# sokunmin/Improved-Body-Parts

Measured on AMD Instinct MI355X. Metric: end-to-end images/sec at 512×512, higher is better.
Workload: dtype f16; 1 GPU; configs[2]+forward: 512x512, flip=on, host->HBM ingest + 4-stage IMHN forward (fp16) + full HIP pafprocess (NMS + limb line-integral + assembly); launch=hipGraph replay, parallelism=image-sharded x1

## Files before the change

improved-body-parts_amd/csrc/posepaf_conv_own.hip:

```cpp
#include <hip/hip_fp16.h>
#include <hip/hip_runtime.h>

#include <atomic>
#include <cstdint>
#include <cstdlib>
#include <type_traits>

#include "../../include/posepaf.h"

namespace {

typedef _Float16 half8_t __attribute__((ext_vector_type(8)));
typedef _Float16 half4_t __attribute__((ext_vector_type(4)));
typedef float float4_t __attribute__((ext_vector_type(4)));

constexpr int BM = 256;
constexpr int NTHREADS = 512;
constexpr int SUB = 1024;

struct ConvParams {
    const _Float16 *x, *w, *bias, *extra, *extra2;
    _Float16 *y, *y2;
    const void *zero;
    int N, H, W, C, K, R, pad, dil, Ho, Wo;
// ... 2 lines not shown
    float *csum;
    int ldy;
    int ldx = 0;
    long M;
    int mode;
    int up;
    float slope;
    int stagger;
    int dbg;
};

__device__ __forceinline__ void lds_dma16(const void *gsrc, unsigned char *lds_wave_base) {
    __builtin_amdgcn_global_load_lds((const __attribute__((address_space(1))) void *)gsrc,
                                     (__attribute__((address_space(3))) void *)lds_wave_base, 16, 0, 0);
}

__device__ __forceinline__ void lds_dma16_buf(__amdgpu_buffer_rsrc_t rsrc, unsigned voffset, unsigned soffset, unsigned char *lds_wave_base) {
    __builtin_amdgcn_raw_ptr_buffer_load_lds(rsrc, (__attribute__((address_space(3))) void *)lds_wave_base, 16, (int)voffset, (int)soffset, 0, 0);
}

typedef float float2_t __attribute__((ext_vector_type(2)));
typedef _Float16 half2_t __attribute__((ext_vector_type(2)));

template <int MODE, int PT, int CT, bool SUMS = false, typename PixelOf>
__device__ __forceinline__ void epilogue_body(const float4_t (&acc)[PT][CT], const ConvParams &p, int lane, int nbase,
                                              PixelOf pixel_of, bool do_store, float *sums_row = nullptr) {
    static_assert(CT % 2 == 0, "channel tiles are finished in pairs");
    const int g = lane >> 4, odd = g & 1, cbase = (g & ~1) * 4;
    const float2_t slope2 = float2_t{p.slope, p.slope};
#pragma unroll
    for (int jp = 0; jp < CT; jp += 2) {
        float csum[8] = {0.f, 0.f, 0.f, 0.f, 0.f, 0.f, 0.f, 0.f};
        const int co = nbase + (jp + odd) * 16 + cbase;
        const half8_t bv = *reinterpret_cast<const half8_t *>(p.bias + co);
        float2_t b2[4];
#pragma unroll
        for (int e = 0; e < 4; e++) b2[e] = float2_t{(float)bv[2 * e], (float)bv[2 * e + 1]};
#pragma unroll
        for (int i = 0; i < PT; i++) {
            float v[8];
#pragma unroll
            for (int e = 0; e < 4; e++) {
                const float a0 = acc[i][jp][e], a1 = acc[i][jp + 1][e];
                const auto sw = __builtin_amdgcn_permlane16_swap(__float_as_uint(a0), __float_as_uint(a1), false, false);
                v[e] = __builtin_bit_cast(float, (unsigned)sw[0]);
                v[4 + e] = __builtin_bit_cast(float, (unsigned)sw[1]);
            }
            const long m = pixel_of(i);
            if (m >= 0) {
                const long o = m * p.K + co;
                half8_t ev = half8_t{0, 0, 0, 0, 0, 0, 0, 0}, ev2 = half8_t{0, 0, 0, 0, 0, 0, 0, 0};
                if (MODE) ev = *reinterpret_cast<const half8_t *>(p.extra + o);
                if (MODE >= 3) ev2 = *reinterpret_cast<const half8_t *>(p.extra2 + o);
                half8_t out, out2;
// ... 72 lines not shown
                v[e] = __builtin_bit_cast(float, (unsigned)sw[0]);
                v[4 + e] = __builtin_bit_cast(float, (unsigned)sw[1]);
            }
            const long m = pixel_of(i);
            keep[i] = half8_t{0, 0, 0, 0, 0, 0, 0, 0};
            if (m >= 0) {
                const half8_t ev = pre[i][jp / 2], ev2 = pre2[i][jp / 2];
                half8_t out, out2;
#pragma unroll
                for (int e = 0; e < 4; e++) {
                    float2_t t = float2_t{v[2 * e], v[2 * e + 1]} + b2[e];
                    const float2_t x = float2_t{(float)ev[2 * e], (float)ev[2 * e + 1]};
                    if (MODE == 1 || MODE == 4) t += x;
                    const float2_t u = t * slope2;
                    t = float2_t{fmaxf(t[0], u[0]), fmaxf(t[1], u[1])};
                    if (MODE == 2) t += x;
                    out[2 * e] = (_Float16)t[0];
                    out[2 * e + 1] = (_Float16)t[1];
                    if (MODE == 4 || MODE == 5) {
                        out2[2 * e] = (_Float16)((float)out[2 * e] + (float)ev2[2 * e]);
                        out2[2 * e + 1] = (_Float16)((float)out[2 * e + 1] + (float)ev2[2 * e + 1]);
                    }
                }
                *reinterpret_cast<half8_t *>(p.y + (m * p.ldy + co)) = out;
                if (MODE == 4 || MODE == 5) *reinterpret_cast<half8_t *>(p.y2 + (m * p.K + co)) = out2;
                keep[i] = (MODE == 4 || MODE == 5) ? out2 : out;
            }
        }
        if (POOL && PT >= 2) {
            constexpr int CB = PT >= 2 ? PT / 2 : 1;
#pragma unroll
            for (int cb = 0; cb < CB; cb++) {
                const half8_t vert = __builtin_elementwise_max(keep[cb], keep[CB + cb]);
                const half8_t pm = __builtin_elementwise_max(vert, lane_xor1(vert));
                if (!(lane & 1)) *reinterpret_cast<half8_t *>(pool + ((pool_base + cb * 8 + ((lane & 15) >> 1)) * p.K + co)) = pm;
            }
        }
    }
}

template <int PT, int CT, typename PixelOf>
__device__ __forceinline__ void epilogue_store(const float4_t (&acc)[PT][CT], const ConvParams &p, int lane, int nbase,
                                               PixelOf pixel_of, bool do_store, float *sums_row = nullptr) {
    if (nbase >= p.K) return;
    if (sums_row) epilogue_body<0, PT, CT, true>(acc, p, lane, nbase, pixel_of, do_store, sums_row);
    else if (p.mode == 0) epilogue_body<0, PT, CT>(acc, p, lane, nbase, pixel_of, do_store);
    else if (p.mode == 1) epilogue_body<1, PT, CT>(acc, p, lane, nbase, pixel_of, do_store);
    else if (p.mode == 2) epilogue_body<2, PT, CT>(acc, p, lane, nbase, pixel_of, do_store);
    else if (p.mode == 3) epilogue_body<3, PT, CT>(acc, p, lane, nbase, pixel_of, do_store);
    else epilogue_body<4, PT, CT>(acc, p, lane, nbase, pixel_of, do_store);
}

template <int PT, int CT, typename PixelOfQ>
__device__ __forceinline__ void epilogue_fullline_probe(const float4_t (&acc)[PT][CT], const ConvParams &p, int lane, int nbase,
                                                        PixelOfQ pixel_of_q) {
    const int co = nbase + (lane >> 3) * 8;
    const half8_t bv = *reinterpret_cast<const half8_t *>(p.bias + co);
#pragma unroll
    for (int jp = 0; jp < CT; jp += 2)
#pragma unroll
        for (int i = 0; i < PT; i++) {
            const long o = pixel_of_q(i * 16 + (jp >> 1) * 8 + (lane & 7)) * p.K + co;
            half8_t out;
#pragma unroll
            for (int e = 0; e < 8; e++) {
                float t = (e < 4 ? acc[i][jp][e] : acc[i][jp + 1][e - 4]) + (float)bv[e];
                t = t > 0.f ? t : t * p.slope;
                out[e] = (_Float16)t;
            }
            *reinterpret_cast<half8_t *>(p.y + o) = out;
        }
}

template <int N>
__device__ __forceinline__ void wait_lgkmcnt() {
    asm volatile("s_waitcnt lgkmcnt(%0)" ::"n"(N) : "memory");
}
__device__ __forceinline__ void mfma_acc(float4_t &c, const half8_t &a, const half8_t &b) {
    asm volatile("v_mfma_f32_16x16x32_f16 %0, %1, %2, %0" : "+v"(c) : "v"(a), "v"(b));
}
template <int OFF>
__device__ __forceinline__ void lds_read16(half8_t &dst, unsigned lds_addr) {
    asm volatile("ds_read_b128 %0, %1 offset:%2" : "=v"(dst) : "v"(lds_addr), "n"(OFF));
}

template <int N>
__device__ __forceinline__ void wait_vmcnt() {
    asm volatile("s_waitcnt vmcnt(%0)" ::"n"(N) : "memory");
}

template <int BN>
__global__ __launch_bounds__(NTHREADS) void k_conv_igemm(const ConvParams p) {
    constexpr int WN = BN / 64;
    constexpr int WM = 8 / WN;
    constexpr int PM = BM / WM;
    constexpr int PT = PM / 16;
    constexpr int CT = 4;
    constexpr int A_BYTES = BM * 32 * 2;
    constexpr int B_BYTES = BN * 32 * 2;
    constexpr int PBUF = A_BYTES + B_BYTES;
    constexpr int NBUF = 4;
    constexpr int BL = BN == 256 ? 2 : 1;
// ... 96 lines not shown
        __builtin_amdgcn_s_setprio(1);
#pragma unroll
        for (int i = 0; i < PT; i++)
#pragma unroll
            for (int j = 0; j < CT; j++) acc[i][j] = __builtin_amdgcn_mfma_f32_16x16x32_f16(wf[j], xf[i], acc[i][j], 0, 0, 0);
        __builtin_amdgcn_s_setprio(0);
        __builtin_amdgcn_s_barrier();
    }
    if (grp == 0) __builtin_amdgcn_s_barrier();

    epilogue_store<PT, CT>(acc, p, lane, n0 + wn * 64, [&](int i) -> long {
        const long m = m0 + wm * PM + i * 16 + (lane & 15);
        if (m >= p.M) return -1;
        if (!p.up_out) return m;
        const int n = (int)(m / HoWo), rem = (int)(m - (long)n * HoWo);
        const int oy_ = rem / p.Wo, ox_ = rem - oy_ * p.Wo;
        return ((long)n * (2 * p.Ho) + 2 * oy_ + p.py) * (2 * p.Wo) + 2 * ox_ + p.px;
    }, true);
}

constexpr int TP = 512;
constexpr int HALO_RES_SUMS = 2048;
constexpr int HALO_DBG_BITS = HALO_RES_SUMS - 1;

struct HaloParams {
    int TW, TH, lgTW;
    int tiles_x, tiles;
    int HWp, nhalo, npieces;
    int gimg, hrows;
    int tps;
};

__device__ unsigned long long g_conv_clk[8 * 512];

template <int BN, int MASK, int LGTW, int PH = -1, int D = 1>
__global__ __launch_bounds__(NTHREADS) void k_conv3x3_halo(const ConvParams p, const HaloParams hp) {
    constexpr int NT = PH < 0 ? 9 : 4;
    static_assert(D == 1 || PH < 0, "the collapsed upsample form has no dilation");
    constexpr int TW = 1 << LGTW, HWp = TW + 2 * D, TH = TP / TW;
    constexpr int dbg = MASK & HALO_DBG_BITS;
    constexpr int WN = BN / 64;
    constexpr int WM = 8 / WN;
    constexpr int PM = TP / WM;
    constexpr int PT = PM / 16;
    constexpr int CT = 4;
    constexpr int WB = BN * 32 * 2;
// ... 81 lines not shown

    const int ncb = p.C / 32;
    const int np = ncb * NT;
    int st_cb = 0, st_tap = 0;
    int st_slot = 0;
    int slot_cur = 0;
    auto stage_w = [&]() {
        lds_dma16_buf(rsrc_of(bw_lo, bw_hi, bw_n), woff, (unsigned)((st_tap * p.C + st_cb * 32) * 2), s_w + st_slot * WB + wave * SUB);
        if (++st_slot == NW) st_slot = 0;
        if (++st_tap == NT) {
            st_tap = 0;
            ++st_cb;
        }
    };
    auto stage_halo = [&](int t, int cb, int buf) {
        lds_dma16_buf(rsrc_of(bx_lo, bx_hi, nx), (unsigned)hsrc[t], (unsigned)(cb * 64), s_halo + buf * halo_bytes + (t * 8 + wave) * SUB);
    };

    const int wfrag = (lane & 15) * 64 + (((lane >> 4) * 16) ^ (((lane & 15) >> 3) << 5));
    const int rows_before = (wm * PM) >> LGTW;
    const int hb0 = ((rows_before + (hp.gimg > 1 ? 2 * (rows_before / p.H) : 0)) * HWp + ((wm * PM) & (TW - 1)) + (lane & 15)) * 64 +
                    (lane >> 4) * 16;
    const unsigned lds_halo = (unsigned)(uintptr_t)(__attribute__((address_space(3))) unsigned char *)s_halo;
    const unsigned lds_w = (unsigned)(uintptr_t)(__attribute__((address_space(3))) unsigned char *)s_w + wn * 4 * SUB;
    unsigned R[4][2];
    auto set_R = [&]() {
#pragma unroll
        for (int k = 0; k < 4; k++) {
            const int M = hb0 + k * 64;
            const unsigned a = lds_halo + (unsigned)(M ^ ((M >> 3) & 32));
            R[k][0] = a;
            R[k][1] = a ^ 32u;
        }
    };
    auto flip_R = [&](int to_buf) {
        const unsigned d = to_buf ? (unsigned)halo_bytes : (unsigned)-halo_bytes;
#pragma unroll
        for (int k = 0; k < 4; k++) R[k][0] += d, R[k][1] += d;
    };
    auto xread = [&](auto TAP, auto I, half8_t &dst) {
        constexpr int tap = decltype(TAP)::value, i = decltype(I)::value;
        constexpr int trow = PH < 0 ? tap / 3 : (PH >> 1) + (tap >> 1), tcol = PH < 0 ? D * (tap % 3) : (PH & 1) + (tap & 1);
        constexpr int Cpix = trow * HWp + tcol + ((i * 16) >> LGTW) * HWp + ((i * 16) & (TW - 1));
        constexpr int C = Cpix * 64, k = Cpix & 3, Chi = C & ~255, f = (Chi >> 8) & 1;
        static_assert(Chi < 65536, "16-bit DS offset");
        lds_read16<Chi>(dst, R[k][f]);
    };

    auto stage_first = [&]() {
        st_cb = 0, st_tap = 0, st_slot = 0;
#pragma unroll
        for (int t = 0; t < NPW; t++)
            if (t < 4 || (t == 4 && p4) || (t == 5 && p5) || (t == 6 && p6)) stage_halo(t, 0, 0);
        for (int q = 0; q < AHEAD && q < np; q++) stage_w();
    };
    unsigned long long acc_t[6] = {0, 0, 0, 0, 0, 0}, t_prev = 0;
    auto stamp = [&](int k) {
        if (dbg & 1024) {
            const unsigned long long t = __builtin_amdgcn_s_memtime();
            if (k >= 0) acc_t[k] += t - t_prev;
            t_prev = t;
        }
    };
    int id = next_tile(blockIdx.x);
    if (id >= total_ids) return;
    for (int z = (int)(blockIdx.x >> 3) * p.stagger / (int)((gridDim.x + 7) >> 3); z > 0; z--) __builtin_amdgcn_s_sleep(127);
    stage_first();
  while (true) {
    const int c_img = n_img, c_ty0 = ty0, c_tx0 = tx0, c_n0 = n0, c_tile = t_idx;
    float4_t acc[PT][CT];
#pragma unroll
    for (int i = 0; i < PT; i++)
#pragma unroll
        for (int j = 0; j < CT; j++) acc[i][j] = float4_t{0.f, 0.f, 0.f, 0.f};
    stamp(-1);
    wait_vmcnt<0>();
    __builtin_amdgcn_s_barrier();
    stamp(0);
    slot_cur = 0;
    half8_t wf[CT], xf[PT];
    set_R();
    lds_read16<0>(wf[0], lds_w + wfrag);
    lds_read16<SUB>(wf[1], lds_w + wfrag);
    using T0 = std::integral_constant<int, 0>;
    xread(T0{}, std::integral_constant<int, 0>{}, xf[0]);
    xread(T0{}, std::integral_constant<int, 1>{}, xf[1]);
    xread(T0{}, std::integral_constant<int, 2>{}, xf[2]);
    xread(T0{}, std::integral_constant<int, 3>{}, xf[3]);
    xread(T0{}, std::integral_constant<int, 4>{}, xf[4]);
    xread(T0{}, std::integral_constant<int, 5>{}, xf[5]);
    xread(T0{}, std::integral_constant<int, 6>{}, xf[6]);
    xread(T0{}, std::integral_constant<int, 7>{}, xf[7]);
// ... 51 lines not shown
                mfma_acc(acc[i][1], wf[1], xf[i]);
            }
        };
        tile_a(std::integral_constant<int, 0>{});
        tile_a(std::integral_constant<int, 1>{});
        tile_a(std::integral_constant<int, 2>{});
        tile_a(std::integral_constant<int, 3>{});
        tile_a(std::integral_constant<int, 4>{});
        tile_a(std::integral_constant<int, 5>{});
        tile_a(std::integral_constant<int, 6>{});
        tile_a(std::integral_constant<int, 7>{});
        static_assert(PT == 8, "eight pixel tiles per wave");
        constexpr bool refill = !(dbg & 4) && !(tap == NT - 1 && !halo);
        if (grp != 0 && !(dbg & 128)) issue_dma();
        if (refill) {
            lds_read16<0>(wf[0], sw_nxt);
            lds_read16<SUB>(wf[1], sw_nxt);
        }
        wait_lgkmcnt<refill ? 2 : 0>();
        if (refill && tap == NT - 1) flip_R((cb + 1) & 1);
        auto tile_b = [&](auto I) {
            constexpr int i = decltype(I)::value;
            if (!(dbg & 2)) {
                mfma_acc(acc[i][2], wf[2], xf[i]);
                mfma_acc(acc[i][3], wf[3], xf[i]);
            }
            if (refill) xread(std::integral_constant<int, ntap>{}, I, xf[i]);
        };
        tile_b(std::integral_constant<int, 0>{});
        tile_b(std::integral_constant<int, 1>{});
        tile_b(std::integral_constant<int, 2>{});
        tile_b(std::integral_constant<int, 3>{});
        tile_b(std::integral_constant<int, 4>{});
        tile_b(std::integral_constant<int, 5>{});
        tile_b(std::integral_constant<int, 6>{});
        tile_b(std::integral_constant<int, 7>{});
        __builtin_amdgcn_s_setprio(0);
        constexpr bool w4 = halo && (NT == 9 ? (tap >= 2 && tap <= 4) : tap <= 1);
        constexpr bool w5 = halo && (NT == 9 ? (tap >= 3 && tap <= 5) : tap <= 1);
        constexpr bool w6 = halo && NPW == 7 && (NT == 9 ? (tap >= 4 && tap <= 6) : tap <= 1);
        const int missing = (w4 && !p4) + (w5 && !p5) + (w6 && !p6);
        static_assert(in_flight >= 3, "the window always holds the three weight slices");
        if (ph + AHEAD >= np) wait_vmcnt<0>();
        else if (missing == 0) wait_vmcnt<in_flight>();
        else if (missing == 1) wait_vmcnt<(in_flight > 1 ? in_flight - 1 : 0)>();
        else if (missing == 2) wait_vmcnt<(in_flight > 2 ? in_flight - 2 : 0)>();
        else wait_vmcnt<(in_flight > 3 ? in_flight - 3 : 0)>();
        __builtin_amdgcn_s_barrier();
// ... 14 lines not shown
    };
    for (int cb = 0; cb + 1 < ncb; cb++) block(std::true_type{}, cb);
    block(std::false_type{}, ncb - 1);
    asm volatile("s_waitcnt lgkmcnt(0)\n\ts_nop 15\n\ts_nop 15" ::: "memory");
    stamp(2);
    if (dbg & 1024) acc_t[5] += __builtin_amdgcn_s_memrealtime() - rt0;

    id = next_tile(id + gridDim.x);
    const bool has_next = id < total_ids;
    if (has_next) stage_first();
    stamp(3);
    if (dbg & 64)
        epilogue_fullline_probe<PT, CT>(acc, p, lane, c_n0 + wn * 64, [&](int qq) -> long {
            const int q = wm * PM + qq;
            const int qy = q >> LGTW, qx = q & (TW - 1);
            return ((long)c_img * p.H + c_ty0 + qy) * p.W + c_tx0 + qx;
        });
    else if constexpr ((MASK & HALO_RES_SUMS) != 0) {
        if (c_n0 + wn * 64 < p.K)
            epilogue_body<1, PT, CT, true>(acc, p, lane, c_n0 + wn * 64, [&](int i) -> long {
                const int q = wm * PM + i * 16 + (lane & 15);
                return ((long)c_img * p.H + c_ty0 + (q >> LGTW)) * p.W + c_tx0 + (q & (TW - 1));
            }, true, p.csum + ((((long)c_img * hp.tiles + c_tile) * WM) / hp.gimg + wm) * p.K);
    } else
    epilogue_store<PT, CT>(acc, p, lane, c_n0 + wn * 64, [&](int i) -> long {
        const int q = wm * PM + i * 16 + (lane & 15);
        const int qy = q >> LGTW, qx = q & (TW - 1);
        if (PH >= 0)
            return (2 * ((long)c_img * p.H + c_ty0 + qy) + (PH >> 1)) * (2 * p.W) + 2 * (c_tx0 + qx) + (PH & 1);
        if (D > 1) {
            const int ry = c_ty0 + qy * D;
            return ry < p.H ? ((long)c_img * p.H + ry) * p.W + c_tx0 + qx : -1;
        }
        return ((long)c_img * p.H + c_ty0 + qy) * p.W + c_tx0 + qx;
    }, !(dbg & 8), p.csum ? p.csum + (((long)c_img * hp.tiles + c_tile) * WM + wm) * p.K : nullptr);
    stamp(4);
    if (!has_next) break;
  }
    if ((dbg & 1024) && threadIdx.x == 0 && blockIdx.x < 512)
        for (int k = 0; k < 6; k++) g_conv_clk[blockIdx.x * 8 + k] = acc_t[k];
}

constexpr int kMaxDevices = 32, kMaxInst = 192;
struct DevState {
    void *zero = nullptr;
    int ncu = 0;
// ... 121 lines not shown
}

template <int PH>
int launch_halo_phase(const ConvParams &p, const HaloParams &g, hipStream_t st) {
    switch (g.lgTW) {
        case 7: return launch_halo_inst<0, 7, PH>(p, g, st);
        case 6: return launch_halo_inst<0, 6, PH>(p, g, st);
        case 5: return launch_halo_inst<0, 5, PH>(p, g, st);
        case 4: return launch_halo_inst<0, 4, PH>(p, g, st);
        default: return PP_ERR_UNSUPPORTED;
    }
}

int launch_halo_res_sums(const ConvParams &p, const HaloParams &g, hipStream_t st) {
    switch (g.lgTW) {
        case 7: return launch_halo_inst<HALO_RES_SUMS, 7>(p, g, st);
        case 6: return launch_halo_inst<HALO_RES_SUMS, 6>(p, g, st);
        case 5: return launch_halo_inst<HALO_RES_SUMS, 5>(p, g, st);
        case 4: return launch_halo_inst<HALO_RES_SUMS, 4>(p, g, st);
        default: return PP_ERR_UNSUPPORTED;
    }
}

int launch_halo(const ConvParams &p, const HaloParams &g, hipStream_t st) {
    switch (p.dbg) {
        case 0: return launch_halo_mask<0>(p, g, st);
#ifdef PP_CONV_DIAG
        case 1: return launch_halo_mask<1>(p, g, st);
        case 4: return launch_halo_mask<4>(p, g, st);
        case 6: return launch_halo_mask<6>(p, g, st);
        case 5: return launch_halo_mask<5>(p, g, st);
        case 7: return launch_halo_mask<7>(p, g, st);
        case 15: return launch_halo_mask<15>(p, g, st);
        case 64: return launch_halo_mask<64>(p, g, st);
        case 71: return launch_halo_mask<71>(p, g, st);
        case 1152: return launch_halo_mask<1152>(p, g, st);
        case 1024: return launch_halo_mask<1024>(p, g, st);
        case 1028: return launch_halo_mask<1028>(p, g, st);
        case 1029: return launch_halo_mask<1029>(p, g, st);
#endif
        default: return PP_ERR_BAD_ARG;
    }
}

template <int BN>
int launch(const ConvParams &p, hipStream_t st) {
// ... 285 lines not shown
                     void *y2, long m, int hw, int c_in, int c_out, int ldy, int extra_mode, float slope, void *stream) {
    return pw_run(x, scale, w, bias, extra, extra2, y, y2, m, hw, c_in, c_out, ldy, extra_mode, slope, nullptr, 0, stream);
}

PP_API int pp_pw_pool_f16(const void *x, const void *scale, const void *w, const void *bias, const void *extra, const void *extra2,
                          void *y, void *y2, void *pool_out, long m, int hw, int width, int c_in, int c_out, int ldy, int extra_mode,
                          float slope, void *stream) {
    if (!pool_out || width <= 0 || hw % width || ((hw / width) & 1) || (reinterpret_cast<uintptr_t>(pool_out) & 15)) return PP_ERR_BAD_ARG;
    if (width % (c_in == 64 ? 64 : 32) || m % hw) return PP_ERR_UNSUPPORTED;
    return pw_run(x, scale, w, bias, extra, extra2, y, y2, m, hw, c_in, c_out, ldy, extra_mode, slope, pool_out, width, stream);
}

PP_API int pp_pw_cat_f16(const void *x, const void *x2, const void *w, const void *bias, const void *extra, void *y, void *pool_out, long m,
                         int hw, int width, int c_in, int c_in2, int c_out, int ldy, int extra_mode, float slope, void *stream) {
    if (!x2 || c_in <= 0 || c_in2 <= 0 || (c_in & 31) || (c_in2 & 31) || (reinterpret_cast<uintptr_t>(x2) & 15) || extra_mode > 2) return PP_ERR_BAD_ARG;
    if (pool_out && (width <= 0 || hw % width || ((hw / width) & 1) || width % (c_in + c_in2 == 64 ? 64 : 32) || m % hw)) return PP_ERR_UNSUPPORTED;
    return pw_run(x, nullptr, w, bias, extra, nullptr, y, nullptr, m, hw, c_in + c_in2, c_out, ldy, extra_mode, slope, pool_out,
                  pool_out ? width : 0, stream, x2, c_in2);
}

static int pw_run(const void *x, const void *scale, const void *w, const void *bias, const void *extra, const void *extra2, void *y,
                  void *y2, long m, int hw, int c_in, int c_out, int ldy, int extra_mode, float slope, void *pool, int width, void *stream,
                  const void *x2, int c_in2, bool pre_form, const void *pre_add) {
    if (!x || !w || !bias || !y || m <= 0 || hw <= 0 || ldy < c_out || extra_mode < 0 || extra_mode == 3 || extra_mode > 5 ||
        (extra_mode != 0 && extra_mode != 5) != (extra != nullptr) || (extra_mode >= 4) != (extra2 != nullptr) ||
        (extra_mode >= 4) != (y2 != nullptr))
        return PP_ERR_BAD_ARG;
    if (!pp_pw_supported(c_in, c_out) || !(slope >= 0.f && slope <= 1.f) || (ldy & 7)) return PP_ERR_UNSUPPORTED;
    if (scale && (hw & 63)) return PP_ERR_UNSUPPORTED;
    const uintptr_t al = reinterpret_cast<uintptr_t>(x) | reinterpret_cast<uintptr_t>(w) | reinterpret_cast<uintptr_t>(bias) |
                         reinterpret_cast<uintptr_t>(extra) | reinterpret_cast<uintptr_t>(extra2) | reinterpret_cast<uintptr_t>(y) |
                         reinterpret_cast<uintptr_t>(y2) | reinterpret_cast<uintptr_t>(scale);
    if (al & 15) return PP_ERR_BAD_ARG;
    PwParams p;
    p.x = static_cast<const _Float16 *>(x);
    p.scale = static_cast<const _Float16 *>(scale);
    p.w = static_cast<const _Float16 *>(w);
    p.e.bias = static_cast<const _Float16 *>(bias);
    p.e.extra = static_cast<const _Float16 *>(extra);
    p.e.extra2 = static_cast<const _Float16 *>(extra2);
    p.e.y = static_cast<_Float16 *>(y);
    p.e.y2 = static_cast<_Float16 *>(y2);
    p.e.K = c_out, p.e.ldy = ldy, p.e.mode = extra_mode, p.e.slope = slope;
    p.M = m, p.Kin = c_in, p.hw = hw;
    p.pool = static_cast<_Float16 *>(pool), p.W = width;
    p.x2 = static_cast<const _Float16 *>(x2), p.kt1 = (c_in - c_in2) / 32;
    int n_split = 1;
// ... 78 lines not shown
                       int upsampled_input, void *stream) {
    return conv_own_run(x, w, bias, extra, extra2, y, y2, n, h, wd, c_in, c_out, ksize, pad, dilation, extra_mode, slope, bn,
                        upsampled_input, c_in, c_out, stream);
}

PP_API int pp_conv_own_ld_f16(const void *x, const void *w, const void *bias, const void *extra, void *y, int n, int h, int wd, int c_in,
                              int c_out, int ksize, int pad, int dilation, int extra_mode, float slope, int bn, int ldx, int ldy,
                              void *stream) {
    if (extra_mode > 2 || ldx < c_in || ldy < c_out || ((ldx | ldy) & 7)) return PP_ERR_BAD_ARG;
    if (bn != 512) return PP_ERR_UNSUPPORTED;
    return conv_own_run(x, w, bias, extra, nullptr, y, nullptr, n, h, wd, c_in, c_out, ksize, pad, dilation, extra_mode, slope, bn, 0,
                        ldx, ldy, stream);
}

static int conv_own_run(const void *x, const void *w, const void *bias, const void *extra, const void *extra2, void *y, void *y2,
                        int n, int h, int wd, int c_in, int c_out, int ksize, int pad, int dilation, int extra_mode, float slope, int bn,
                        int upsampled_input, int ldx, int ldy, void *stream) {
    if (!x || !w || !bias || !y || n <= 0 || h <= 0 || wd <= 0 || ksize <= 0 || pad < 0 || dilation <= 0 || extra_mode < 0 ||
        extra_mode > 4 || (extra_mode != 0) != (extra != nullptr) || (extra_mode >= 3) != (extra2 != nullptr) ||
        (extra_mode == 4) != (y2 != nullptr) || (upsampled_input != 0 && upsampled_input != 1) ||
        ((reinterpret_cast<uintptr_t>(extra2) | reinterpret_cast<uintptr_t>(y2)) & 15))
        return PP_ERR_BAD_ARG;
    if ((upsampled_input || extra_mode == 3) && bn != 512) return PP_ERR_UNSUPPORTED;
    if (upsampled_input && ((h | wd) & 1)) return PP_ERR_BAD_ARG;
    if (!pp_conv_own_supported(c_in, c_out, ksize)) return PP_ERR_UNSUPPORTED;
    if (!(slope >= 0.f && slope <= 1.f)) return PP_ERR_UNSUPPORTED;
    const uintptr_t al = reinterpret_cast<uintptr_t>(x) | reinterpret_cast<uintptr_t>(w) | reinterpret_cast<uintptr_t>(bias) |
                         reinterpret_cast<uintptr_t>(extra) | reinterpret_cast<uintptr_t>(y);
    if (al & 15) return PP_ERR_BAD_ARG;
    const int ho = h + 2 * pad - dilation * (ksize - 1), wo = wd + 2 * pad - dilation * (ksize - 1);
    if (ho <= 0 || wo <= 0) return PP_ERR_BAD_ARG;
    if (bn != 0 && bn != 512 && ((bn != 256 && bn != 128 && bn != 64) || c_out % bn)) return PP_ERR_UNSUPPORTED;
    hipStream_t st = static_cast<hipStream_t>(stream);
    DevState *ds = dev_state();
    if (!ds) return PP_ERR_HIP;
    if (!ds->zero) {
        if (capturing(st)) return PP_ERR_UNSUPPORTED;
        if (hipMalloc(&ds->zero, 256) != hipSuccess || hipMemset(ds->zero, 0, 256) != hipSuccess) return PP_ERR_HIP;
    }
    ConvParams p;
    p.x = static_cast<const _Float16 *>(x);
    p.w = static_cast<const _Float16 *>(w);
    p.bias = static_cast<const _Float16 *>(bias);
    p.extra = static_cast<const _Float16 *>(extra);
    p.extra2 = static_cast<const _Float16 *>(extra2);
    p.up = upsampled_input;
    p.y = static_cast<_Float16 *>(y);
    p.y2 = static_cast<_Float16 *>(y2);
    p.zero = ds->zero;
    p.N = n; p.H = h; p.W = wd; p.C = c_in; p.K = c_out; p.R = ksize; p.pad = pad; p.dil = dilation; p.Ho = ho; p.Wo = wo;
    p.ldy = ldy;
    p.ldx = ldx;
    p.csum = nullptr;
    p.pad_y = p.pad_x = pad, p.up_out = 0, p.py = p.px = 0;
    p.M = (long)n * ho * wo;
    p.mode = extra_mode;
    p.slope = slope;
#ifdef PP_CONV_DIAG
    static const int dbg = std::getenv("POSEPAF_CONV_DBG") ? std::atoi(std::getenv("POSEPAF_CONV_DBG")) : 0;
    p.dbg = dbg;
#else
    p.dbg = 0;
#endif
    static const int stagger = std::getenv("POSEPAF_CONV_STAGGER") ? std::atoi(std::getenv("POSEPAF_CONV_STAGGER")) : -1;
    p.stagger = stagger;
    if (bn == 0 || bn == 512) {
        HaloParams g;
        if (halo_geometry(p, g)) return launch_halo(p, g, st);
        if (bn != 0 || ldx != c_in || ldy != c_out) return PP_ERR_UNSUPPORTED;
        bn = c_out % 256 == 0 ? 256 : (c_out % 128 == 0 ? 128 : 64);
    }
    switch (bn) {
        case 256: return launch<256>(p, st);
        case 128: return launch<128>(p, st);
        default: return launch<64>(p, st);
    }
}

PP_API int pp_conv_own_sums_splits(int h, int wd) {
    ConvParams q;
    q.R = 3, q.pad = 1, q.dil = 1, q.C = 32, q.K = 128, q.H = h, q.W = wd, q.N = 1, q.csum = nullptr;
    HaloParams g;
    return (halo_geometry(q, g) && g.gimg == 1) ? g.tiles * 4 : 0;
}
PP_API int pp_conv_own_sums_f16(const void *x, const void *w, const void *bias, void *y, void *sums_ws, int n, int h, int wd, int c_in,
                                int c_out, float slope, void *stream) {
    if (!x || !w || !bias || !y || !sums_ws || n <= 0 || h <= 0 || wd <= 0) return PP_ERR_BAD_ARG;
    if (!pp_conv_own_supported(c_in, c_out, 3) || !(slope >= 0.f && slope <= 1.f)) return PP_ERR_UNSUPPORTED;
// ... 104 lines not shown
```

improved-body-parts_amd/posepaf/fused_model.py:

```python
from __future__ import annotations

import os

import torch
import torch.nn.functional as F
from torch import nn

LEAK = 0.01
USE_PWCONV = False
USE_FUSED_CONV = True
USE_OWN_CONV = True
TUNE_MIOPEN = os.environ.get("POSEPAF_TUNE_MIOPEN", "0") == "1"
OWN_VARIANTS = {101: 256, 102: 128, 103: 64, 104: 512}
UP2_COLLAPSED_BN = (256, 128, 64, 512)
PW_VARIANT = 105
USE_PW = True
USE_SUM_FUSION = True
USE_SLICE_OUTPUT = True
USE_COLLAPSED_UP2 = True
USE_FOLDED_MERGE = True
USE_CAT_SKIP = True
USE_SE_KERNEL = True
USE_POOL_FUSION = True
USE_RES_SUM_FUSION = True
USE_PRE_FUSION = True
PW_TUNE_MAX_CIN = 704
_conv_choice: dict = {}
_conv_timing: dict = {}
_conv_calls: dict = {}
_TUNE_REPS = 5
OWN_MARGIN = 0.03


_progress = None


def set_progress(fn) -> None:
    global _progress
    _progress = fn


def _timed(fn):
    fn()
    torch.cuda.synchronize()
    ts = []
    for _ in range(_TUNE_REPS):
        e0, e1 = torch.cuda.Event(enable_timing=True), torch.cuda.Event(enable_timing=True)
        e0.record()
# ... 749 lines not shown
    return FConv(m.conv, m.bn, m.relu is not None if act is None else act)


class FResidual(nn.Module):
    def __init__(self, r):
        super().__init__()
        cb = r.convBlock
        self.c1 = FConv(cb[0], cb[1], True)
        self.c2 = FConv(cb[3], cb[4], True)
        self.c3 = FConv(cb[6], cb[7], False)
        self.c3.act = r.relu_flag
        self.skip = FConv(r.skipConv[0], r.skipConv[1], False) if r.ins != r.outs else None
        if self.skip is not None:
            self.c3.bias = nn.Parameter(self.c3.bias + self.skip.bias, requires_grad=False)

    def forward(self, x, out=None):
        if self.skip is not None and out is None:
            y = self._cat(x, False)
            if y is not None:
                return y[0]
        res = self.skip.conv_only(x) if self.skip is not None else x
        return self.c3(self.c2(self.c1(x)), res, out=out)

    def forward_pool(self, x):
        if self.skip is not None:
            y = self._cat(x, True)
            if y is not None:
                return y
        res = self.skip.conv_only(x) if self.skip is not None else x
        return self.c3.forward_pool(self.c2(self.c1(x)), res)

    def _cat_fused(self, x, want_pool, pool_ok):
        from . import _lib
        if not (USE_PW and USE_CAT_SKIP and USE_OWN_CONV and x.is_cuda and x.dtype == torch.float16):
            return None
        k, c1 = self.c3.weight.shape[:2]
        c2 = self.skip.weight.shape[1]
        n, _, h, w = x.shape
        if (tuple(self.skip.weight.shape[2:]) != (1, 1) or self.skip.stride != (1, 1)
                or not _lib.load().pp_pw_supported(c1 + c2, k) or c1 % 32 or c2 % 32):
            return None
        if getattr(self, "_wcat", None) is None or self._wcat.device != x.device:
            self._wcat = torch.cat([self.c3.weight.detach().flatten(1), self.skip.weight.detach().flatten(1)], dim=1).contiguous()

        def run():
            t = _cl(self.c2(self.c1(x)))
            xx, y = _cl(x), self.c3._out(x, h, w)
            pooled = self.c3._out(x, h // 2, w // 2) if pool_ok else None
            rc = _lib.load().pp_pw_cat_f16(_ptr(t), _ptr(xx), _ptr(self._wcat), _ptr(self.c3.bias), None, _ptr(y), _ptr(pooled), n * h * w,
                                           h * w, w if pool_ok else 0, c1, c2, k, k, 0, self.c3._slope, _stream(x))
            if rc != 0:
                return None
            return y, (pooled if pool_ok else (maxpool2(y) if want_pool else None))
        return run

    def _cat(self, x, want_pool):
        k, c1 = self.c3.weight.shape[:2]
        c2 = self.skip.weight.shape[1]
        n, _, h, w = x.shape
        pool_ok = want_pool and USE_POOL_FUSION and h % 2 == 0 and w % (64 if c1 + c2 == 64 else 32) == 0 and c1 + c2 <= 512
        run = self._cat_fused(x, want_pool, pool_ok)
        if run is None:
            return None
        key = ("cat", n, c1, c2, h, w, k, bool(self.c3.act), pool_ok)

        def separate():
            res = self.skip.conv_only(x)
            t = self.c2(self.c1(x))
            return self.c3.forward_pool(t, res) if want_pool else (self.c3(t, res), None)

        return run() if _choose(key, True, [(0, "separate", separate), (1, "fused", run)]) else None


class FHourglass(nn.Module):
    def __init__(self, hg):
        super().__init__()
        self.depth = hg.depth
        self.levels = nn.ModuleList()
        for i in range(hg.depth):
            mods = [FResidual(hg.hg[i][0]), FResidual(hg.hg[i][1]), FResidual(hg.hg[i][2]), _fconv_from_block(hg.hg[i][3])]
            if i == hg.depth - 1:
                mods.append(FResidual(hg.hg[i][4]))
            self.levels.append(nn.ModuleList(mods))

# ... 80 lines not shown
        self.mpred = nn.ModuleList([nn.ModuleList([_fconv_from_block(m.conv) for m in ms]) for ms in p.merge_preds])
        self.folded_merge = bool(USE_FOLDED_MERGE)
        for t_, (mf, mp) in enumerate(zip(self.mfeat, self.mpred)):
            for s_, (f, q) in enumerate(zip(mf, mp)):
                f.bias = nn.Parameter(f.bias + q.bias, requires_grad=False)
                if self.folded_merge:
                    hd = self.head[t_][s_]
                    wp = q.weight.detach().float().flatten(1)
                    wh = hd.weight.detach().float().flatten(1)
                    f.weight = nn.Parameter((f.weight.detach().float().flatten(1) + wp @ wh).view_as(f.weight), requires_grad=False)
                    f.bias = nn.Parameter(f.bias.detach().float() + wp @ hd.bias.detach().float(), requires_grad=False)
                wq = torch.zeros((q.weight.shape[0], 64, 1, 1), dtype=q.weight.dtype)
                wq[:, : q.weight.shape[1]] = q.weight.detach()
                q.w_in64 = nn.Parameter(wq, requires_grad=False)

    @classmethod
    def from_network(cls, net):
        if cls is FusedIMHN:
            from models import posenet_final
            if isinstance(net.posenet, posenet_final.PoseNet):
                return FusedIMHNFinal(net)
        return cls(net)

    def forward(self, imgs, stage_preds: bool = False, all_preds: bool = False):
        seen = []
        x = imgs.permute(0, 3, 1, 2)
        x = self.stem(x)
        pooled = self.res1.forward_pool(x)[1]
        if USE_SLICE_OUTPUT and pooled.is_cuda and pooled.dtype == torch.float16:
            c2 = self.res2.c3.weight.shape[0]
            cd = self.dil[-1].weight.shape[0]
            n, _, h, w = pooled.shape
            buf = torch.empty((n, c2 + cd, h, w), dtype=pooled.dtype, device=pooled.device, memory_format=torch.channels_last)
            d = self.res2(pooled, out=buf[:, :c2])
            for i, m in enumerate(self.dil):
                d = m(d, out=buf[:, c2:] if i == len(self.dil) - 1 else None)
            x = buf
        else:
            x = self.res2(pooled)
            d = x
            for m in self.dil:
                d = m(d)
            x = torch.cat([x, d], dim=1)
        caches, x_pooled = None, None
        for t in range(self.S):
            last = t == self.S - 1
            scales = range(1) if last and not all_preds else range(self.K)
            hg = self.hg[t](x, None if caches is None else caches[0], x_pooled)
            if caches is not None:
                hg = [hg[0]] + [hg[s] + caches[s] for s in scales if s > 0]
            feats = [self.feat[t][s](hg[s], fold=True) for s in scales]
            if last or stage_preds or all_preds or not self.folded_merge:
                preds = [self.head[t][s](feats[s]) for s in (scales if all_preds or not self.folded_merge else range(1))]
                seen.append(preds if all_preds else preds[0])
            if last:
                return seen if stage_preds or all_preds else preds[0]
            if self.folded_merge:
                c0, x, x_pooled = self.mfeat[t][0].forward_dual(feats[0], None, x, want_pool=True)
                caches = [c0] + [self.mfeat[t][s](feats[s]) for s in scales if s > 0]
                continue
            mp = [self._merge_pred(t, s, preds[s]) for s in scales]
            c0, x, x_pooled = self.mfeat[t][0].forward_dual(feats[0], mp[0], x, want_pool=True)
            caches = [c0] + [self.mfeat[t][s](feats[s], mp[s]) for s in scales if s > 0]

    def _merge_pred(self, t, s, pred):
        q, padded = self.mpred[t][s], self.head[t][s].last_padded
        if padded is not None and padded.shape[1] == 64:
            return F.conv2d(padded, q.w_in64)
        return q.conv_only(pred)

# ... 36 lines not shown
        super().__init__()
        self.c1, self.c2, self.c3 = _fconv_from_block(seq[0]), _fconv_from_block(seq[1]), _fconv_from_block(seq[2])

    def forward(self, h, gains, cache=None):
        return self.c3(self.c2(self.c1.forward_pre(h, gains, cache)))


class FusedIMHNFinal(FusedIMHN):

    def __init__(self, net):
        nn.Module.__init__(self)
        p = net.posenet
        self.S, self.K = p.nstack, 5
        pre = p.pre
        self.stem = FStem(pre.conv1, pre.bn1, True)
        self.res1, self.res2, self.res3 = FResidual(pre.res1), FResidual(pre.res2), FResidual(pre.res3)
        self.hg = nn.ModuleList([FHourglassFinal(h) for h in p.hourglass])
        self.att = nn.ModuleList([nn.ModuleList([FSE(se) for se in ses]) for ses in p.channel_attention])
        self.feat = nn.ModuleList([nn.ModuleList([FFeatureFinal(s) for s in f.before_regress]) for f in p.features])
        self._init_heads_and_merges(p)

    def forward(self, imgs, stage_preds: bool = False, all_preds: bool = False):
        seen = []
        x = self.stem(imgs.permute(0, 3, 1, 2))
        x, x_pooled = self.res3.forward_pool(self.res2(self.res1.forward_pool(x)[1]))
        caches = None
        for t in range(self.S):
            last = t == self.S - 1
            scales = range(1) if last and not all_preds else range(self.K)
            hg = self.hg[t](x, x_pooled, scales)
            feats = [self.feat[t][s](hg[s][0], self.att[t][s].gains(hg[s][0], hg[s][1]), None if caches is None else caches[s])
                     for s in scales]
            if last or stage_preds or all_preds or not self.folded_merge:
                preds = [self.head[t][s](feats[s]) for s in (scales if all_preds or not self.folded_merge else range(1))]
                seen.append(preds if all_preds else preds[0])
            if last:
                return seen if stage_preds or all_preds else preds[0]
            if self.folded_merge:
                c0, x, x_pooled = self.mfeat[t][0].forward_dual(feats[0], None, x, want_pool=True)
                caches = [c0] + [self.mfeat[t][s](feats[s]) for s in scales if s > 0]
                continue
            mp = [self._merge_pred(t, s, preds[s]) for s in scales]
            c0, x, x_pooled = self.mfeat[t][0].forward_dual(feats[0], mp[0], x, want_pool=True)
            caches = [c0] + [self.mfeat[t][s](feats[s], mp[s]) for s in scales if s > 0]


class GraphedForward:

    def __init__(self, module, example: torch.Tensor, warmup: int = 3):
        self.module = module
        self.static_in = example.clone()
        s = torch.cuda.Stream()
# ... 28 lines not shown
```

Measured before the change: 981.1 images/sec.

## Prune dead multi-scale branches, add pool-only residual output and half-width conv tiles

Only the scale-0 prediction of the last stage is returned by default, so scales 1-4 of every stage are now skipped once an input shape has been seen (and during graph capture). The first call for each shape still runs the full set so tuning covers every conv. The first residual block now writes only its max-pooled output and skips the full-resolution store, since only the pooled tensor is consumed. A new halo-conv variant (bn=576) handles channel counts that leave a 64-wide remainder: the tail tile skips the upper pair of MFMAs and stores only half the tile, avoiding wasted tensor-core work. The pruning relies on those skipped scales truly being dead when neither stage_preds nor all_preds is requested.

New measurement: 1107 images/sec, median of 6. +12.8%, better.

```diff
diff --git a/improved-body-parts_amd/csrc/posepaf_conv_own.hip b/improved-body-parts_amd/csrc/posepaf_conv_own.hip
--- a/improved-body-parts_amd/csrc/posepaf_conv_own.hip
+++ b/improved-body-parts_amd/csrc/posepaf_conv_own.hip
@@ -48,14 +48,14 @@
 typedef float float2_t __attribute__((ext_vector_type(2)));
 typedef _Float16 half2_t __attribute__((ext_vector_type(2)));
 
-template <int MODE, int PT, int CT, bool SUMS = false, typename PixelOf>
+template <int MODE, int PT, int CT, bool SUMS = false, int CTU = CT, typename PixelOf>
 __device__ __forceinline__ void epilogue_body(const float4_t (&acc)[PT][CT], const ConvParams &p, int lane, int nbase,
                                               PixelOf pixel_of, bool do_store, float *sums_row = nullptr) {
-    static_assert(CT % 2 == 0, "channel tiles are finished in pairs");
+    static_assert(CT % 2 == 0 && CTU % 2 == 0 && CTU <= CT, "channel tiles are finished in pairs");
     const int g = lane >> 4, odd = g & 1, cbase = (g & ~1) * 4;
     const float2_t slope2 = float2_t{p.slope, p.slope};
 #pragma unroll
-    for (int jp = 0; jp < CT; jp += 2) {
+    for (int jp = 0; jp < CTU; jp += 2) {
         float csum[8] = {0.f, 0.f, 0.f, 0.f, 0.f, 0.f, 0.f, 0.f};
         const int co = nbase + (jp + odd) * 16 + cbase;
         const half8_t bv = *reinterpret_cast<const half8_t *>(p.bias + co);
@@ -174,7 +174,7 @@
                         out2[2 * e + 1] = (_Float16)((float)out[2 * e + 1] + (float)ev2[2 * e + 1]);
                     }
                 }
-                *reinterpret_cast<half8_t *>(p.y + (m * p.ldy + co)) = out;
+                if (!POOL || p.y) *reinterpret_cast<half8_t *>(p.y + (m * p.ldy + co)) = out;
                 if (MODE == 4 || MODE == 5) *reinterpret_cast<half8_t *>(p.y2 + (m * p.K + co)) = out2;
                 keep[i] = (MODE == 4 || MODE == 5) ? out2 : out;
             }
@@ -191,16 +191,16 @@
     }
 }
 
-template <int PT, int CT, typename PixelOf>
+template <int PT, int CT, int CTU = CT, typename PixelOf>
 __device__ __forceinline__ void epilogue_store(const float4_t (&acc)[PT][CT], const ConvParams &p, int lane, int nbase,
                                                PixelOf pixel_of, bool do_store, float *sums_row = nullptr) {
     if (nbase >= p.K) return;
-    if (sums_row) epilogue_body<0, PT, CT, true>(acc, p, lane, nbase, pixel_of, do_store, sums_row);
-    else if (p.mode == 0) epilogue_body<0, PT, CT>(acc, p, lane, nbase, pixel_of, do_store);
-    else if (p.mode == 1) epilogue_body<1, PT, CT>(acc, p, lane, nbase, pixel_of, do_store);
-    else if (p.mode == 2) epilogue_body<2, PT, CT>(acc, p, lane, nbase, pixel_of, do_store);
-    else if (p.mode == 3) epilogue_body<3, PT, CT>(acc, p, lane, nbase, pixel_of, do_store);
-    else epilogue_body<4, PT, CT>(acc, p, lane, nbase, pixel_of, do_store);
+    if (sums_row) epilogue_body<0, PT, CT, true, CTU>(acc, p, lane, nbase, pixel_of, do_store, sums_row);
+    else if (p.mode == 0) epilogue_body<0, PT, CT, false, CTU>(acc, p, lane, nbase, pixel_of, do_store);
+    else if (p.mode == 1) epilogue_body<1, PT, CT, false, CTU>(acc, p, lane, nbase, pixel_of, do_store);
+    else if (p.mode == 2) epilogue_body<2, PT, CT, false, CTU>(acc, p, lane, nbase, pixel_of, do_store);
+    else if (p.mode == 3) epilogue_body<3, PT, CT, false, CTU>(acc, p, lane, nbase, pixel_of, do_store);
+    else epilogue_body<4, PT, CT, false, CTU>(acc, p, lane, nbase, pixel_of, do_store);
 }
 
 template <int PT, int CT, typename PixelOfQ>
@@ -230,6 +230,12 @@
 }
 __device__ __forceinline__ void mfma_acc(float4_t &c, const half8_t &a, const half8_t &b) {
     asm volatile("v_mfma_f32_16x16x32_f16 %0, %1, %2, %0" : "+v"(c) : "v"(a), "v"(b));
+}
+__device__ __forceinline__ void mfma_pair_unless(float4_t &c0, float4_t &c1, const half8_t &a0, const half8_t &a1, const half8_t &b, int skip) {
+    asm volatile("s_cmp_lg_u32 %5, 0\n\ts_cbranch_scc1 .Lpp_skip%=\n\tv_mfma_f32_16x16x32_f16 %0, %2, %4, %0\n\tv_mfma_f32_16x16x32_f16 %1, %3, %4, %1\n.Lpp_skip%=:"
+                 : "+v"(c0), "+v"(c1)
+                 : "v"(a0), "v"(a1), "v"(b), "s"(skip)
+                 : "scc");
 }
 template <int OFF>
 __device__ __forceinline__ void lds_read16(half8_t &dst, unsigned lds_addr) {
@@ -372,6 +378,7 @@
 constexpr int TP = 512;
 constexpr int HALO_RES_SUMS = 2048;
 constexpr int HALO_DBG_BITS = HALO_RES_SUMS - 1;
+constexpr int HALO_HALF = 4096;
 
 struct HaloParams {
     int TW, TH, lgTW;
@@ -499,7 +506,7 @@
     const int hb0 = ((rows_before + (hp.gimg > 1 ? 2 * (rows_before / p.H) : 0)) * HWp + ((wm * PM) & (TW - 1)) + (lane & 15)) * 64 +
                     (lane >> 4) * 16;
     const unsigned lds_halo = (unsigned)(uintptr_t)(__attribute__((address_space(3))) unsigned char *)s_halo;
-    const unsigned lds_w = (unsigned)(uintptr_t)(__attribute__((address_space(3))) unsigned char *)s_w + wn * 4 * SUB;
+    const unsigned lds_w_full = (unsigned)(uintptr_t)(__attribute__((address_space(3))) unsigned char *)s_w + wn * 4 * SUB;
     unsigned R[4][2];
     auto set_R = [&]() {
 #pragma unroll
@@ -545,6 +552,9 @@
     stage_first();
   while (true) {
     const int c_img = n_img, c_ty0 = ty0, c_tx0 = tx0, c_n0 = n0, c_tile = t_idx;
+    const int half_s = (MASK & HALO_HALF) ? __builtin_amdgcn_readfirstlane(c_n0 + 64 >= p.K ? 1 : 0) : 0;
+    const bool half = half_s != 0;
+    const unsigned lds_w = half ? lds_w_full - wn * 2 * SUB : lds_w_full;
     float4_t acc[PT][CT];
 #pragma unroll
     for (int i = 0; i < PT; i++)
@@ -642,8 +652,11 @@
         auto tile_b = [&](auto I) {
             constexpr int i = decltype(I)::value;
             if (!(dbg & 2)) {
-                mfma_acc(acc[i][2], wf[2], xf[i]);
-                mfma_acc(acc[i][3], wf[3], xf[i]);
+                if constexpr ((MASK & HALO_HALF) != 0) mfma_pair_unless(acc[i][2], acc[i][3], wf[2], wf[3], xf[i], half_s);
+                else {
+                    mfma_acc(acc[i][2], wf[2], xf[i]);
+                    mfma_acc(acc[i][3], wf[3], xf[i]);
+                }
             }
             if (refill) xread(std::integral_constant<int, ntap>{}, I, xf[i]);
         };
@@ -704,6 +717,11 @@
                 const int q = wm * PM + i * 16 + (lane & 15);
                 return ((long)c_img * p.H + c_ty0 + (q >> LGTW)) * p.W + c_tx0 + (q & (TW - 1));
             }, true, p.csum + ((((long)c_img * hp.tiles + c_tile) * WM) / hp.gimg + wm) * p.K);
+    } else if (half) {
+        epilogue_store<PT, CT, 2>(acc, p, lane, c_n0 + wn * 32, [&](int i) -> long {
+            const int q = wm * PM + i * 16 + (lane & 15);
+            return ((long)c_img * p.H + c_ty0 + (q >> LGTW)) * p.W + c_tx0 + (q & (TW - 1));
+        }, true);
     } else
     epilogue_store<PT, CT>(acc, p, lane, c_n0 + wn * 64, [&](int i) -> long {
         const int q = wm * PM + i * 16 + (lane & 15);
@@ -871,6 +889,16 @@
     }
 }
 
+int launch_halo_half(const ConvParams &p, const HaloParams &g, hipStream_t st) {
+    switch (g.lgTW) {
+        case 7: return launch_halo_inst<HALO_HALF, 7>(p, g, st);
+        case 6: return launch_halo_inst<HALO_HALF, 6>(p, g, st);
+        case 5: return launch_halo_inst<HALO_HALF, 5>(p, g, st);
+        case 4: return launch_halo_inst<HALO_HALF, 4>(p, g, st);
+        default: return PP_ERR_UNSUPPORTED;
+    }
+}
+
 int launch_halo(const ConvParams &p, const HaloParams &g, hipStream_t st) {
     switch (p.dbg) {
         case 0: return launch_halo_mask<0>(p, g, st);
@@ -1202,7 +1230,7 @@
 static int pw_run(const void *x, const void *scale, const void *w, const void *bias, const void *extra, const void *extra2, void *y,
                   void *y2, long m, int hw, int c_in, int c_out, int ldy, int extra_mode, float slope, void *pool, int width, void *stream,
                   const void *x2, int c_in2, bool pre_form, const void *pre_add) {
-    if (!x || !w || !bias || !y || m <= 0 || hw <= 0 || ldy < c_out || extra_mode < 0 || extra_mode == 3 || extra_mode > 5 ||
+    if (!x || !w || !bias || (!y && !pool) || m <= 0 || hw <= 0 || ldy < c_out || extra_mode < 0 || extra_mode == 3 || extra_mode > 5 ||
         (extra_mode != 0 && extra_mode != 5) != (extra != nullptr) || (extra_mode >= 4) != (extra2 != nullptr) ||
         (extra_mode >= 4) != (y2 != nullptr))
         return PP_ERR_BAD_ARG;
@@ -1327,6 +1355,8 @@
         ((reinterpret_cast<uintptr_t>(extra2) | reinterpret_cast<uintptr_t>(y2)) & 15))
         return PP_ERR_BAD_ARG;
     if ((upsampled_input || extra_mode == 3) && bn != 512) return PP_ERR_UNSUPPORTED;
+    if (bn == 576 && (c_out % 128 != 64 || ksize != 3 || pad != 1 || dilation != 1 || extra_mode > 2 || ldx != c_in || ldy != c_out))
+        return PP_ERR_UNSUPPORTED;
     if (upsampled_input && ((h | wd) & 1)) return PP_ERR_BAD_ARG;
     if (!pp_conv_own_supported(c_in, c_out, ksize)) return PP_ERR_UNSUPPORTED;
     if (!(slope >= 0.f && slope <= 1.f)) return PP_ERR_UNSUPPORTED;
@@ -1335,7 +1365,7 @@
     if (al & 15) return PP_ERR_BAD_ARG;
     const int ho = h + 2 * pad - dilation * (ksize - 1), wo = wd + 2 * pad - dilation * (ksize - 1);
     if (ho <= 0 || wo <= 0) return PP_ERR_BAD_ARG;
-    if (bn != 0 && bn != 512 && ((bn != 256 && bn != 128 && bn != 64) || c_out % bn)) return PP_ERR_UNSUPPORTED;
+    if (bn != 0 && bn != 512 && bn != 576 && ((bn != 256 && bn != 128 && bn != 64) || c_out % bn)) return PP_ERR_UNSUPPORTED;
     hipStream_t st = static_cast<hipStream_t>(stream);
     DevState *ds = dev_state();
     if (!ds) return PP_ERR_HIP;
@@ -1369,6 +1399,10 @@
 #endif
     static const int stagger = std::getenv("POSEPAF_CONV_STAGGER") ? std::atoi(std::getenv("POSEPAF_CONV_STAGGER")) : -1;
     p.stagger = stagger;
+    if (bn == 576) {
+        HaloParams g;
+        return halo_geometry(p, g) ? launch_halo_half(p, g, st) : PP_ERR_UNSUPPORTED;
+    }
     if (bn == 0 || bn == 512) {
         HaloParams g;
         if (halo_geometry(p, g)) return launch_halo(p, g, st);
diff --git a/improved-body-parts_amd/posepaf/fused_model.py b/improved-body-parts_amd/posepaf/fused_model.py
--- a/improved-body-parts_amd/posepaf/fused_model.py
+++ b/improved-body-parts_amd/posepaf/fused_model.py
@@ -11,7 +11,7 @@
 USE_FUSED_CONV = True
 USE_OWN_CONV = True
 TUNE_MIOPEN = os.environ.get("POSEPAF_TUNE_MIOPEN", "0") == "1"
-OWN_VARIANTS = {101: 256, 102: 128, 103: 64, 104: 512}
+OWN_VARIANTS = {101: 256, 102: 128, 103: 64, 104: 512, 106: 576}
 UP2_COLLAPSED_BN = (256, 128, 64, 512)
 PW_VARIANT = 105
 USE_PW = True
@@ -24,6 +24,8 @@
 USE_POOL_FUSION = True
 USE_RES_SUM_FUSION = True
 USE_PRE_FUSION = True
+USE_PRUNED_SCALES = True
+USE_POOL_ONLY = True
 PW_TUNE_MAX_CIN = 704
 _conv_choice: dict = {}
 _conv_timing: dict = {}
@@ -819,15 +821,15 @@
         res = self.skip.conv_only(x) if self.skip is not None else x
         return self.c3(self.c2(self.c1(x)), res, out=out)
 
-    def forward_pool(self, x):
+    def forward_pool(self, x, pooled_only: bool = False):
         if self.skip is not None:
-            y = self._cat(x, True)
+            y = self._cat(x, True, pooled_only and USE_POOL_ONLY)
             if y is not None:
                 return y
         res = self.skip.conv_only(x) if self.skip is not None else x
         return self.c3.forward_pool(self.c2(self.c1(x)), res)
 
-    def _cat_fused(self, x, want_pool, pool_ok):
+    def _cat_fused(self, x, want_pool, pool_ok, pooled_only=False):
         from . import _lib
         if not (USE_PW and USE_CAT_SKIP and USE_OWN_CONV and x.is_cuda and x.dtype == torch.float16):
             return None
@@ -842,7 +844,7 @@
 
         def run():
             t = _cl(self.c2(self.c1(x)))
-            xx, y = _cl(x), self.c3._out(x, h, w)
+            xx, y = _cl(x), (None if pooled_only and pool_ok else self.c3._out(x, h, w))
             pooled = self.c3._out(x, h // 2, w // 2) if pool_ok else None
             rc = _lib.load().pp_pw_cat_f16(_ptr(t), _ptr(xx), _ptr(self._wcat), _ptr(self.c3.bias), None, _ptr(y), _ptr(pooled), n * h * w,
                                            h * w, w if pool_ok else 0, c1, c2, k, k, 0, self.c3._slope, _stream(x))
@@ -851,12 +853,12 @@
             return y, (pooled if pool_ok else (maxpool2(y) if want_pool else None))
         return run
 
-    def _cat(self, x, want_pool):
+    def _cat(self, x, want_pool, pooled_only=False):
         k, c1 = self.c3.weight.shape[:2]
         c2 = self.skip.weight.shape[1]
         n, _, h, w = x.shape
         pool_ok = want_pool and USE_POOL_FUSION and h % 2 == 0 and w % (64 if c1 + c2 == 64 else 32) == 0 and c1 + c2 <= 512
-        run = self._cat_fused(x, want_pool, pool_ok)
+        run = self._cat_fused(x, want_pool, pool_ok, pooled_only)
         if run is None:
             return None
         key = ("cat", n, c1, c2, h, w, k, bool(self.c3.act), pool_ok)
@@ -983,11 +985,24 @@
                 return FusedIMHNFinal(net)
         return cls(net)
 
+    def _prune_scales(self, imgs, all_preds) -> bool:
+        if all_preds or not USE_PRUNED_SCALES:
+            return False
+        if not imgs.is_cuda or _capturing():
+            return True
+        tuned = self.__dict__.setdefault("_tuned_inputs", set())
+        key = (imgs.device, imgs.dtype, tuple(imgs.shape))
+        if key in tuned:
+            return True
+        tuned.add(key)
+        return False
+
     def forward(self, imgs, stage_preds: bool = False, all_preds: bool = False):
         seen = []
+        prune = self._prune_scales(imgs, all_preds)
         x = imgs.permute(0, 3, 1, 2)
         x = self.stem(x)
-        pooled = self.res1.forward_pool(x)[1]
+        pooled = self.res1.forward_pool(x, pooled_only=True)[1]
         if USE_SLICE_OUTPUT and pooled.is_cuda and pooled.dtype == torch.float16:
             c2 = self.res2.c3.weight.shape[0]
             cd = self.dil[-1].weight.shape[0]
@@ -1006,7 +1021,7 @@
         caches, x_pooled = None, None
         for t in range(self.S):
             last = t == self.S - 1
-            scales = range(1) if last and not all_preds else range(self.K)
+            scales = range(1) if (last or prune) and not all_preds else range(self.K)
             hg = self.hg[t](x, None if caches is None else caches[0], x_pooled)
             if caches is not None:
                 hg = [hg[0]] + [hg[s] + caches[s] for s in scales if s > 0]
@@ -1089,12 +1104,13 @@
 
     def forward(self, imgs, stage_preds: bool = False, all_preds: bool = False):
         seen = []
+        prune = self._prune_scales(imgs, all_preds)
         x = self.stem(imgs.permute(0, 3, 1, 2))
-        x, x_pooled = self.res3.forward_pool(self.res2(self.res1.forward_pool(x)[1]))
+        x, x_pooled = self.res3.forward_pool(self.res2(self.res1.forward_pool(x, pooled_only=True)[1]))
         caches = None
         for t in range(self.S):
             last = t == self.S - 1
-            scales = range(1) if last and not all_preds else range(self.K)
+            scales = range(1) if (last or prune) and not all_preds else range(self.K)
             hg = self.hg[t](x, x_pooled, scales)
             feats = [self.feat[t][s](hg[s][0], self.att[t][s].gains(hg[s][0], hg[s][1]), None if caches is None else caches[s])
                      for s in scales]
```
